# efeslab/Atom

Measured on AMD Instinct MI355X. Metric: effective TOPS, W4A4 group-128 GEMM + 128 INT8 outlier cols, fp16 out, higher is better.
Workload: dtype int4xint4 exact integer dot (BF6-coded on the f8f6f4 MFMA; INT8 MFMA for the keeper), fp32 dequant, fp16 out

## Files before the change

### atom_amd/csrc/gemm_w4a4_f6.hip

```cpp
#include <type_traits>
#include "common.h"
#include "quant_math.h"

namespace atom {

__global__ void splitk_reduce_kernel(const float *ws, half_t *D, int64_t MN, int splits);

namespace f6 {

typedef const __attribute__((address_space(1))) void *gptr_t;
typedef __attribute__((address_space(3))) void *lptr_t;
typedef int v8i __attribute__((ext_vector_type(8)));
typedef float v16f __attribute__((ext_vector_type(16)));

constexpr int TN = 2;
constexpr int PITCH = 104;
constexpr float kMagic = 12582912.0f;
constexpr int kMagicBits = 0x4B400000;

template <int BM_, int BN_, int TM_, int NS_, int OCC_ = 2, int FS_ = 0>
struct Cfg {
  static constexpr int FS = FS_;
  static constexpr int FS32 = FS_ == 1;
  static constexpr int OCC = OCC_;
// ... 221 lines not shown
      for (int q = 0; q < 4; ++q) sbp[q] = *reinterpret_cast<const v2u *>(psb + (tn * 32 + 8 * q) * 2);
#pragma unroll
      for (int r = 0; r < 16; ++r) {
        const half_t *hv = reinterpret_cast<const half_t *>(&sbp[r >> 2]);
        const float idot = __int_as_float(a[r]) - kMagic;
        c[tn][tm][r] = __builtin_fmaf(idot, (float)hv[r & 3] * sa, c[tn][tm][r]);
        asm volatile("" : "+v"(c[tn][tm][r]));
      }
    }
  }
}

template <class C, bool SK, int ABL = 0>
__global__ __launch_bounds__(C::NT, C::OCC) void gemm_w4a4_f6_kernel(GemmParams p) {
  extern __shared__ __attribute__((aligned(16))) char lds[];
  constexpr int TM = C::TM, NS = C::NS;
  const int tid = threadIdx.x;
  const int lane = tid & 63;
  const int wave = __builtin_amdgcn_readfirstlane(tid >> 6);
  __builtin_assume(wave >= 0 && wave < C::NW);
  const int wm = wave / C::WGN, wn = wave % C::WGN;

  const int nbn = (p.N + C::BN - 1) / C::BN, nbm = (p.M + C::BM - 1) / C::BM;
  const int nwg = nbm * nbn;
  int id = blockIdx.x;
  {
    const int q = nwg >> 3, r = nwg & 7, xcd = id & 7, k = id >> 3;
    id = (xcd < r ? xcd * (q + 1) : r * (q + 1) + (xcd - r) * q) + k;
  }
  constexpr int GM = 4;
  const int band = id / (GM * nbn), inband = id % (GM * nbn);
  const int rows_in_band = min(GM, nbm - band * GM);
  const int bm = band * GM + inband % rows_in_band, bn = inband / rows_in_band;
  const int m0 = bm * C::BM, n0 = bn * C::BN;

  float c[TN][TM][16];
#pragma unroll
  for (int a = 0; a < TN; ++a)
#pragma unroll
    for (int b = 0; b < TM; ++b)
#pragma unroll
      for (int r = 0; r < 16; ++r) c[a][b][r] = 0.f;

  const int csteps = p.G + 1;
  const int s_begin = SK ? (int)((int64_t)csteps * blockIdx.y / p.splits) : 0;
  const int c_end = SK ? (int)((int64_t)csteps * (blockIdx.y + 1) / p.splits) : csteps;
  const bool has_keeper = c_end == csteps;
  const int nsteps = c_end + (has_keeper ? 1 : 0);
  auto issue = [&](int step) {
    char *slot = lds + (step % NS) * C::STAGE_BYTES;
    const int s = min(step, nsteps - 1);
    if (wave >= C::NDW) return;
    if (s < p.G) issue_int4<C>(p, s, slot, wave, lane, m0, n0);
    else issue_keeper<C>(p, s - p.G, slot, wave, lane, m0, n0);
  };
#pragma unroll
  for (int s = 0; s < NS - 1; ++s) issue(s_begin + s);
  unsigned long long *tbase = nullptr;
  if constexpr ((ABL & 16) != 0)
    if (blockIdx.x == 0 && lane == 0) tbase = reinterpret_cast<unsigned long long *>(p.Dsz) + wave * 64 * 8;
#define ATOM_F6_STAMP(k) if constexpr ((ABL & 16) != 0) { if (tbase) tbase[step * 8 + k] = __builtin_amdgcn_s_memtime(); }
#define ATOM_F6_STEP(ISSUE, COMPUTE)                                                     \
  {                                                                                      \
    ATOM_F6_STAMP(0)                                                                     \
    asm volatile("s_waitcnt vmcnt(%0)" ::"n"((ABL & 1) ? 0 : C::GLDS * (NS - 2)) : "memory"); \
    ATOM_F6_STAMP(1)                                                                     \
    __builtin_amdgcn_s_barrier();                                                        \
    ATOM_F6_STAMP(2)                                                                     \
    ISSUE;                                                                               \
    __builtin_amdgcn_sched_barrier(0);                                                   \
    COMPUTE;                                                                             \
  }
  int step = s_begin;
  for (; step + NS - 1 < min(p.G, nsteps); ++step) {
    char *nslot = lds + ((step + NS - 1) % NS) * C::STAGE_BYTES;
    const int g = step + NS - 1;
    auto dma = [&](int i) { if (!(ABL & 1) && wave < C::NDW) issue_int4_piece<C>(p, g, nslot, wave, lane, m0, n0, i); };
    ATOM_F6_STEP((void)0, (compute_int4<C, ABL>(lds + (step % NS) * C::STAGE_BYTES, wm, wn, lane, c, dma, tbase ? tbase + step * 8 : nullptr, wave < C::NW / 2)))
  }
  for (; step < min(p.G, nsteps); ++step)
    ATOM_F6_STEP(if (!(ABL & 1)) issue(step + NS - 1), (compute_int4<C, ABL>(lds + (step % NS) * C::STAGE_BYTES, wm, wn, lane, c, NoDma(), nullptr, wave < C::NW / 2)))
  __builtin_amdgcn_s_setprio(0);
#undef ATOM_F6_STEP
  if (has_keeper) {
    asm volatile("s_waitcnt vmcnt(0)" ::: "memory");
    __builtin_amdgcn_s_barrier();
    if constexpr (NS == 2) {
      if (wave < C::NDW) issue_keeper<C>(p, 1, lds + ((p.G + 1) % NS) * C::STAGE_BYTES, wave, lane, m0, n0);
      asm volatile("s_waitcnt vmcnt(0)" ::: "memory");
      __builtin_amdgcn_s_barrier();
    }
    compute_keeper<C>(lds + (p.G % NS) * C::STAGE_BYTES, lds + ((p.G + 1) % NS) * C::STAGE_BYTES, wm, wn, lane, c);
    ++step;
  }
  { ATOM_F6_STAMP(0) }
  asm volatile("s_waitcnt vmcnt(0)" ::: "memory");
  __builtin_amdgcn_s_barrier();

  const int l31 = lane & 31, h = lane >> 5;
  if constexpr (SK) {
    float *wsp = p.ws + (int64_t)blockIdx.y * p.M * p.N;
#pragma unroll
    for (int tm = 0; tm < TM; ++tm) {
      const int m = m0 + wm * C::WM + tm * 32 + l31;
      if (m >= p.M) continue;
#pragma unroll
      for (int tn = 0; tn < TN; ++tn)
#pragma unroll
        for (int q = 0; q < 4; ++q) {
          const int n = n0 + wn * 64 + tn * 32 + 8 * q + 4 * h;
          if (n >= p.N) continue;
          *reinterpret_cast<v4f *>(wsp + (int64_t)m * p.N + n) =
              v4f{c[tn][tm][4 * q], c[tn][tm][4 * q + 1], c[tn][tm][4 * q + 2], c[tn][tm][4 * q + 3]};
        }
    }
    return;
  }
  constexpr int EP_STRIDE = 144;
  char *ep = lds + wave * (64 * EP_STRIDE);
#pragma unroll
  for (int half = 0; half < TM / 2; ++half) {
#pragma unroll
    for (int t2 = 0; t2 < 2; ++t2) {
      const int tm = half * 2 + t2;
#pragma unroll
      for (int tn = 0; tn < TN; ++tn)
#pragma unroll
        for (int q = 0; q < 4; ++q) {
          v2u o;
          half_t *ov = reinterpret_cast<half_t *>(&o);
#pragma unroll
          for (int k = 0; k < 4; ++k) ov[k] = f2h(c[tn][tm][4 * q + k]);
          *reinterpret_cast<v2u *>(ep + (t2 * 32 + l31) * EP_STRIDE + (tn * 32 + 8 * q + 4 * h) * 2) = o;
        }
    }
#pragma unroll
    for (int i = 0; i < 8; ++i) {
      const int rl = i * 8 + (lane >> 3);
      const int ch = lane & 7;
      const v4u v = *reinterpret_cast<const v4u *>(ep + rl * EP_STRIDE + ch * 16);
      const int m = m0 + wm * C::WM + half * 64 + rl;
      const int n = n0 + wn * 64 + ch * 8;
      if (m < p.M && n < p.N) *reinterpret_cast<v4u *>(p.D + (int64_t)m * p.N + n) = v;
    }
  }
}

typedef float v4f_t __attribute__((ext_vector_type(4)));

template <bool PAIR, bool INTER = true>
__device__ __forceinline__ void deq_pair(const v4f_t &a0, const v4f_t &a1, float sa, const float *sb, float (&c0)[4], float (&c1)[4]) {
  if constexpr (PAIR) {
    static_assert(INTER, "shared products need the interleaved rows");
    float s[4];
#pragma unroll
    for (int r = 0; r < 4; ++r) s[r] = sa * sb[r];
#pragma unroll
    for (int r = 0; r < 4; ++r) { c0[r] = __builtin_fmaf(a0[r], s[r], c0[r]); asm volatile("" : "+v"(c0[r])); }
#pragma unroll
    for (int r = 0; r < 4; ++r) { c1[r] = __builtin_fmaf(a1[r], s[r], c1[r]); asm volatile("" : "+v"(c1[r])); }
  } else if constexpr (INTER) {
    float s[8];
#pragma unroll
    for (int k = 0; k < 2; ++k)
#pragma unroll
      for (int r = 0; r < 4; ++r) s[4 * k + r] = sa * sb[2 * r + k];
#pragma unroll
    for (int r = 0; r < 4; ++r) { c0[r] = __builtin_fmaf(a0[r], s[r], c0[r]); asm volatile("" : "+v"(c0[r])); }
#pragma unroll
    for (int r = 0; r < 4; ++r) { c1[r] = __builtin_fmaf(a1[r], s[4 + r], c1[r]); asm volatile("" : "+v"(c1[r])); }
  } else {
    float s[4];
#pragma unroll
    for (int r = 0; r < 4; ++r) s[r] = sa * sb[r];
#pragma unroll
    for (int r = 0; r < 4; ++r) { c0[r] = __builtin_fmaf(a0[r], s[r], c0[r]); asm volatile("" : "+v"(c0[r])); }
#pragma unroll
    for (int r = 0; r < 4; ++r) s[r] = sa * sb[4 + r];
#pragma unroll
    for (int r = 0; r < 4; ++r) { c1[r] = __builtin_fmaf(a1[r], s[r], c1[r]); asm volatile("" : "+v"(c1[r])); }
  }
}

__device__ __forceinline__ void dequant4x(const v4f_t &acc, float sa, const v2u &sb, float (&c)[4]) {
  const half_t *hv = reinterpret_cast<const half_t *>(&sb);
  float t[4];
#pragma unroll
  for (int r = 0; r < 4; ++r) t[r] = (float)hv[r] * sa;
#pragma unroll
  for (int r = 0; r < 4; ++r) {
    c[r] = __builtin_fmaf(acc[r], t[r], c[r]);
    asm volatile("" : "+v"(c[r]));
  }
}

template <class C, class F = NoDma, bool PRIO = (C::NW >= 8), bool PH = false>
__device__ __forceinline__ void compute_int4_x16(const char *slot, int wm, int wn, int lane, float (&c)[4][C::WM / 16][4], F dma = F(),
                                                 bool older = false, unsigned *tp = nullptr) {
  const int l15 = lane & 15, kb = lane >> 4;
  const char *pw = slot + (wn * 64 + l15) * PITCH + kb * 24;
  constexpr int NTB = C::WM / 16;
  const char *pa = slot + C::A_OFF + (wm * C::WM + l15) * PITCH + kb * 24;
  const char *psa = slot + C::A_OFF + (wm * C::WM + l15) * PITCH + 96;
  const char *psb = slot + C::SB_OFF + (wn * 64 + 4 * kb) * (C::FS32 ? 4 : 2);
  v8i af[4], bf[2];
  using sa_t = typename std::conditional<C::FS != 0, float, half_t>::type;
  using sb_t = typename std::conditional<C::FS != 0, v4f_t, v2u>::type;
  constexpr int SA_AT = C::FS ? 4 : 0;
  sb_t sb[4];
  bf[0] = frag24(pa);
  af[0] = frag24(pw);
  sa_t sah = *reinterpret_cast<const sa_t *>(psa + SA_AT);
#pragma unroll
  for (int fb = 1; fb < 4; ++fb) af[fb] = frag24(pw + fb * 16 * PITCH);
#pragma unroll
  for (int fb = 0; fb < 4; ++fb) {
    if constexpr (C::FS == 2) {
      const v2u raw = *reinterpret_cast<const v2u *>(psb + fb * 32);
      const half_t *hv = reinterpret_cast<const half_t *>(&raw);
      sb[fb] = v4f_t{(float)hv[0], (float)hv[1], (float)hv[2], (float)hv[3]};
    } else {
      sb[fb] = *reinterpret_cast<const sb_t *>(psb + fb * (C::FS32 ? 64 : 32));
    }
  }
  constexpr int GS = 2, NG = 4 * NTB / GS, GPB = 4 / GS, DEPTH = 1;
  v4f_t acc[DEPTH + 1][GS];
  auto mma = [&](int g) {
    const int tb = g / GPB, f0 = (g % GPB) * GS;
#pragma unroll
    for (int k = 0; k < GS; ++k) {
      acc[g % (DEPTH + 1)][k] = v4f_t{0.f, 0.f, 0.f, 0.f};
      if constexpr (C::FS)
        acc[g % (DEPTH + 1)][k] = __builtin_amdgcn_mfma_scale_f32_16x16x128_f8f6f4(af[f0 + k], bf[tb & 1], acc[g % (DEPTH + 1)][k], 3, 3, 0, 0, 0, 0);
      else
        acc[g % (DEPTH + 1)][k] = __builtin_amdgcn_mfma_scale_f32_16x16x128_f8f6f4(af[f0 + k], bf[tb & 1], acc[g % (DEPTH + 1)][k], 3, 3, 0, 127, 0, 127);
    }
  };
  mma(0);
#ifdef ATOM_TOOLS
  if (tp) { __builtin_amdgcn_sched_barrier(0); tp[0] = (unsigned)__builtin_amdgcn_s_memtime(); }
#endif
  float sa = 0.f;
#pragma unroll
  for (int g = 0; g < NG; ++g) {
    const int tb = g / GPB, f0 = (g % GPB) * GS;
    __builtin_amdgcn_sched_barrier(0);
#ifdef ATOM_TOOLS
    if (tp && g == NG / 2) tp[1] = (unsigned)__builtin_amdgcn_s_memtime();
#endif
    if (g % GPB == 0) {
      sa = (float)sah;
      if (tb + 1 < NTB) {
        bf[(tb + 1) & 1] = frag24(pa + (tb + 1) * 16 * PITCH);
        sah = *reinterpret_cast<const sa_t *>(psa + SA_AT + (tb + 1) * 16 * PITCH);
      }
      if constexpr (PH) {
        if (tb == NTB / 2) __builtin_amdgcn_s_barrier();
      }
      if constexpr (PRIO) {
        if (tb == 0) { if (older) __builtin_amdgcn_s_setprio(0); else __builtin_amdgcn_s_setprio(2); }
        if (tb == NTB / 2) { if (older) __builtin_amdgcn_s_setprio(2); else __builtin_amdgcn_s_setprio(0); }
      }
    }
    if (g + DEPTH < NG) mma(g + DEPTH);
    if (g % GPB == GPB - 1) {
#pragma unroll
      for (int i = (tb * C::GLDS + NTB - 1) / NTB; i < ((tb + 1) * C::GLDS + NTB - 1) / NTB; ++i) dma(i);
    }
    __builtin_amdgcn_sched_barrier(0);
    {
      float w[4 * GS];
#pragma unroll
      for (int k = 0; k < GS; ++k)
#pragma unroll
        for (int r = 0; r < 4; ++r) {
          if constexpr (C::FS) w[4 * k + r] = sb[f0 + k][r];
          else w[4 * k + r] = (float)reinterpret_cast<const half_t *>(&sb[f0 + k])[r];
        }
      deq_pair<false, false>(acc[g % (DEPTH + 1)][0], acc[g % (DEPTH + 1)][1], sa, w, c[f0][tb], c[f0 + 1][tb]);
    }
  }
}

template <class C, bool PH = false>
__device__ __forceinline__ void compute_keeper_x16(const char *slot, const char *slot1, int wm, int wn, int lane, float (&c)[4][C::WM / 16][4]) {
  const int l15 = lane & 15, kb = lane >> 4;
  const int sw = (l15 >> 2) & 3;
  const int ow = (wn * 64 + l15) * 64 + ((kb ^ sw) << 4);
  constexpr int NTB = C::WM / 16;
  const int oa = (C::BN + wm * C::WM + l15) * 64 + ((kb ^ sw) << 4);
  const char *psa = slot + C::KP_SA_OFF + (wm * C::WM + l15) * 4;
  const char *psb = slot + C::SB_OFF + (wn * 64 + 4 * kb) * 2;
  v4i af[4], af1[4];
  v2u sb[4];
#pragma unroll
  for (int fb = 0; fb < 4; ++fb) {
    af[fb] = __builtin_bit_cast(v4i, *reinterpret_cast<const v4u *>(slot + ow + fb * 1024));
    af1[fb] = __builtin_bit_cast(v4i, *reinterpret_cast<const v4u *>(slot1 + ow + fb * 1024));
    sb[fb] = *reinterpret_cast<const v2u *>(psb + fb * 32);
  }
#pragma unroll
  for (int tb = 0; tb < NTB; ++tb) {
    if constexpr (PH) {
      if (tb == NTB / 2) __builtin_amdgcn_s_barrier();
    }
    const v4i b = __builtin_bit_cast(v4i, *reinterpret_cast<const v4u *>(slot + oa + tb * 1024));
    const v4i b1 = __builtin_bit_cast(v4i, *reinterpret_cast<const v4u *>(slot1 + oa + tb * 1024));
    const float sa = (float)*reinterpret_cast<const half_t *>(psa + tb * 64);
#pragma unroll
    for (int fb = 0; fb < 4; ++fb) {
      v4i a = {0, 0, 0, 0};
      a = __builtin_amdgcn_mfma_i32_16x16x64_i8(af[fb], b, a, 0, 0, 0);
      a = __builtin_amdgcn_mfma_i32_16x16x64_i8(af1[fb], b1, a, 0, 0, 0);
      const v4f_t f = {(float)a[0], (float)a[1], (float)a[2], (float)a[3]};
      dequant4x(f, sa, sb[fb], c[fb][tb]);
    }
  }
}

template <class C, int KG>
__device__ __forceinline__ void kg_exchange_store(const GemmParams &p, char *lds_all, float (&c)[4][C::WM / 16][4], int kg, int wave, int wm,
                                                  int wn, int lane, int m0, int n0) {
  constexpr int NTB = C::WM / 16, EP_STRIDE = 144;
  const int l15 = lane & 15, kb = lane >> 4;
  const int wave_all = kg * C::NW + wave;
  constexpr int HB = NTB / 2, XF = HB * 16;
  float *xw = reinterpret_cast<float *>(lds_all + C::NW * KG * (HB * 16 * EP_STRIDE)) + (kg * C::NW + wave) * XF * 64 + lane;
  const float *xr = reinterpret_cast<const float *>(lds_all + C::NW * KG * (HB * 16 * EP_STRIDE)) + ((1 - kg) * C::NW + wave) * XF * 64 + lane;
#pragma unroll
  for (int h = 0; h < 2; ++h)
    if (h != kg) {
#pragma unroll
      for (int t = 0; t < HB; ++t)
#pragma unroll
// ... 449 lines not shown
    const int q = nwg >> 3, r = nwg & 7, xcd = id & 7, k = id >> 3;
    id = (xcd < r ? xcd * (q + 1) : r * (q + 1) + (xcd - r) * q) + k;
  }
  constexpr int GM = 4;
  const int band = id / (GM * nbn), inband = id % (GM * nbn);
  const int rows_in_band = min(GM, nbm - band * GM);
  const int bm = band * GM + inband % rows_in_band, bn = inband / rows_in_band;
  const int m0 = bm * C::BM, n0 = bn * C::BN;

  float c[4][8][4];
#pragma unroll
  for (int a = 0; a < 4; ++a)
#pragma unroll
    for (int b = 0; b < 8; ++b)
#pragma unroll
      for (int r = 0; r < 4; ++r) c[a][b][r] = 0.f;

  const int G = p.G;
  auto slot_of = [&](int stage) { return lds + (stage % 3) * C::STAGE_BYTES; };
  auto issue = [&](int stage) {
    if (stage < G) issue_int4<C>(p, stage, slot_of(stage), wave, lane, m0, n0);
    else if (stage < G + 2) issue_keeper<C>(p, stage - G, slot_of(stage), wave, lane, m0, n0);
  };
  issue(0);
  issue(1);
  kstamp(1);
  asm volatile("s_waitcnt vmcnt(%0)" ::"n"(C::GLDS) : "memory");
  __builtin_amdgcn_s_barrier();
  kstamp(2);
  const int l15 = lane & 15, kb = lane >> 4;
  PRegs<C> R;
  R.lo[0] = l15 * (2 * PITCH) + kb * 24;
  R.lo[1] = R.lo[0] + 8;
  R.lo[2] = R.lo[0] + 16;
  asm volatile("" : "+v"(R.lo[1]));
  asm volatile("" : "+v"(R.lo[2]));
  {
    const char *slot = slot_of(0);
    const char *pw = slot + wn * 64 * PITCH, *pa = slot + C::A_OFF + wm * 128 * PITCH;
    const char *psa = pa + l15 * (2 * PITCH) + 96;
    R.bf[2] = frag3<C>(R, pa, p_row(0) * PITCH);
#pragma unroll
    for (int fb = 0; fb < 4; ++fb) R.af[fb] = frag3<C>(R, pw, p_row(fb) * PITCH);
    R.bf[1] = frag3<C>(R, pa, p_row(1) * PITCH);
    R.bf[0] = R.bf[1];
    R.sah[2] = *reinterpret_cast<const half_t *>(psa + p_row(0) * PITCH);
    R.sah[1] = *reinterpret_cast<const half_t *>(psa + p_row(1) * PITCH);
    R.sah[0] = (half_t)0;
    p_load_sb<C>(R, slot, wn, kb);
    p_cvt_sb<C>(R, 0);
    p_cvt_sb<C>(R, 1);
#pragma unroll
    for (int k = 0; k < 2; ++k) R.acc[1][k] = v4f_t{0.f, 0.f, 0.f, 0.f};
#pragma unroll
    for (int t = 0; t < 8; ++t) R.sa[t] = 0.f;
  }
  auto sync = [&]() {
    asm volatile("s_waitcnt vmcnt(0)" ::: "memory");
    if constexpr (!(ABL & 512)) __builtin_amdgcn_s_barrier();
  };
  {
    int s = 0;
    auto dma4 = [&](int i) { if (i < C::GLDS) issue_int4_piece<C>(p, s + 2, slot_of(s + 2), wave, lane, m0, n0, i); };
    auto dmak0 = [&](int i) { if (i == 0) issue_keeper<C>(p, 0, slot_of(G), wave, lane, m0, n0); };
    auto dmak1 = [&](int i) { if (i == 0) issue_keeper<C>(p, 1, slot_of(G + 1), wave, lane, m0, n0); };
    auto tr_sel = [&]() {
      if constexpr ((ABL & 16) != 0) {
        if (tr_on) tr_i += 6;
        tr_on = blockIdx.x == 0 && tr_i + 6 <= 78 && (s < 3 || s == G / 2 || s == G / 2 + 1 || s + 3 >= G);
      }
    };
    kstamp(3);
    if constexpr ((ABL & 1024) != 0) {
      auto dma4f = [&](int i) { if (i < C::GLDS) issue_int4_piece<C>(p, s + 2, lds + 2 * C::STAGE_BYTES, wave, lane, m0, n0, i); };
      for (; s + 2 < G; ++s) p_step<C, false, ABL>(R, lds, lds + C::STAGE_BYTES, wm, wn, lane, c, sync, dma4f, stamp);
    }
    for (; s + 2 < G; ++s) { tr_sel(); p_step<C, false, ABL>(R, slot_of(s), slot_of(s + 1), wm, wn, lane, c, sync, dma4, stamp); }
    if (G >= 2) { tr_sel(); p_step<C, false, ABL>(R, slot_of(s), slot_of(s + 1), wm, wn, lane, c, sync, dmak0, stamp); ++s; }
    tr_sel();
    p_step<C, true, ABL>(R, slot_of(s), slot_of(s + 1), wm, wn, lane, c, sync, dmak1, stamp);
  }
  kstamp(4);
  p_drain<C>(R, c);
  kstamp(5);
  asm volatile("s_waitcnt vmcnt(0)" ::: "memory");
  __builtin_amdgcn_s_barrier();
  kstamp(6);
  if constexpr (!(ABL & 128)) p_keeper<C>(slot_of(G), slot_of(G + 1), wm, wn, lane, c);
  kstamp(7);

#pragma unroll
  for (int tb = 0; tb < 8; ++tb) {
    const int m = m0 + wm * 128 + p_row(tb) + 2 * l15;
    if (m >= p.M) continue;
#pragma unroll
    for (int h = 0; h < 2; ++h) {
      const int n = n0 + wn * 64 + 32 * h + 8 * kb;
      if (n >= p.N) continue;
      v4u o;
      half_t *ov = reinterpret_cast<half_t *>(&o);
#pragma unroll
      for (int r = 0; r < 4; ++r) {
        ov[2 * r] = f2h(c[2 * h][tb][r]);
        ov[2 * r + 1] = f2h(c[2 * h + 1][tb][r]);
      }
      if constexpr ((ABL & 64) != 0) { if (o.x != 0x12345678u) continue; }
      *reinterpret_cast<v4u *>(p.D + (int64_t)m * p.N + n) = o;
    }
  }
  if constexpr ((ABL & 16) != 0) {
    kstamp(8);
    asm volatile("s_waitcnt vmcnt(0)" ::: "memory");
    kstamp(9);
    if (blockIdx.x == 0) {
      if (lane == 0) trl[79] = (unsigned)__builtin_amdgcn_s_memrealtime();
      asm volatile("s_waitcnt lgkmcnt(0)" ::: "memory");
      for (int i = lane; i < 80; i += 64) reinterpret_cast<unsigned *>(p.Dsz)[wave * 80 + i] = trl[i];
    }
  }
}

template <class C>
struct QC {
  static constexpr int SB_OFF = C::SB_OFF;
  static constexpr int STAGE = C::SB_OFF + C::BN * 4;
  static constexpr int LDS_BYTES = 3 * STAGE;
  static_assert(LDS_BYTES <= 160 * 1024 && STAGE + (32 * 3 + 1) * PITCH + 100 < 65536, "q kernel: stage layout / ds offsets");
};

typedef float v2f_t __attribute__((ext_vector_type(2)));
#ifdef ATOM_SA_B32
struct QSa {
  float v;
  __device__ __forceinline__ QSa() = default;
  __device__ __forceinline__ QSa(float f) : v(f) {}
  __device__ __forceinline__ operator float() const { return v; }
};
#else
struct QSa {
  v2f_t p;
  __device__ __forceinline__ QSa() = default;
  __device__ __forceinline__ QSa(float f) : p{0.f, f} {}
  __device__ __forceinline__ QSa(v2f_t q) : p(q) {}
  __device__ __forceinline__ operator float() const { asm volatile("" ::"v"(p)); return p.y; }
};
#endif

template <class C, bool PAIR = false, bool SA2 = false>
struct QRegs {
  v8i af[4];
  v8i bf[3];
  float sb[2][PAIR ? 4 : 8];
  QSa sa[4];
  v2f_t sa2[2];
  v4f_t acc[2][2];
  int aW[2][3], aA[2][3], aS[2], aB[2];
  int aS2[3][4];
  __device__ __forceinline__ float tscale(int tb) const {
    if constexpr (SA2) return sa2[(tb & 3) >> 1][tb & 1];
    else return sa[tb & 3];
  }
#ifdef ATOM_F6_PAIR128
  int aWp[2][3];
#endif
};

template <int SL> __device__ __forceinline__ constexpr int q_set() { return SL == 2 ? 1 : 0; }
template <class C, int SL> __device__ __forceinline__ constexpr int q_imm() { return SL == 1 ? QC<C>::STAGE : 0; }

template <class T>
__device__ __forceinline__ T q_ld0(int a, int imm) {
#if defined(__HIP_DEVICE_COMPILE__)
  typedef const __attribute__((address_space(3))) char *cp_t;
  typedef const __attribute__((address_space(3))) T *tp_t;
  return *(tp_t)((cp_t)(unsigned)a + imm);
#else
  return T{};
#endif
}
template <class C, int SL, bool Z = false>
__device__ __forceinline__ v8i q_frag(const char *lds, const int (&a)[2][3], int off, int ro) {
  const char *b = lds + (SL < 0 ? ro : q_imm<C, SL>()) + off;
  v2u x, y, z;
  if constexpr (Z) {
    const int imm = (SL < 0 ? 0 : q_imm<C, SL>()) + off, r = SL < 0 ? ro : 0;
    x = q_ld0<v2u>(a[q_set<SL>()][0] + r, imm);
    y = q_ld0<v2u>(a[q_set<SL>()][1] + r, imm);
    z = q_ld0<v2u>(a[q_set<SL>()][2] + r, imm);
  } else {
    x = *reinterpret_cast<const v2u *>(b + a[q_set<SL>()][0]);
    y = *reinterpret_cast<const v2u *>(b + a[q_set<SL>()][1]);
    z = *reinterpret_cast<const v2u *>(b + a[q_set<SL>()][2]);
  }
  asm volatile("" ::: "memory");
  return v8i{(int)x.x, (int)x.y, (int)y.x, (int)y.y, (int)z.x, (int)z.y, 0, 0};
}
#ifdef ATOM_F6_PAIR128
template <class C, int SL>
__device__ __forceinline__ void q_frag_pair(const char *lds, const int (&a)[2][3], int off, int ro, v8i &f0, v8i &f1) {
  const char *b = lds + (SL < 0 ? ro : q_imm<C, SL>()) + off;
  const v4u x = *reinterpret_cast<const v4u *>(b + a[q_set<SL>()][0]);
  const v4u y = *reinterpret_cast<const v4u *>(b + a[q_set<SL>()][1]);
  const v4u z = *reinterpret_cast<const v4u *>(b + a[q_set<SL>()][2]);
  asm volatile("" ::: "memory");
  f0 = v8i{(int)x.x, (int)x.y, (int)y.x, (int)y.y, (int)z.x, (int)z.y, 0, 0};
  f1 = v8i{(int)x.z, (int)x.w, (int)y.z, (int)y.w, (int)z.z, (int)z.w, 0, 0};
}
#endif
template <class C, int SL, class RG>
__device__ __forceinline__ QSa q_scale(const char *lds, const RG &R, int off, int ro) {
#ifdef ATOM_SA_B32
  return *reinterpret_cast<const float *>(lds + (SL < 0 ? ro : q_imm<C, SL>()) + off + R.aS[q_set<SL>()] + 4);
#else
  return QSa(*reinterpret_cast<const v2f_t *>(lds + (SL < 0 ? ro : q_imm<C, SL>()) + off + R.aS[q_set<SL>()]));
#endif
}
template <class C, int SL, class RG>
__device__ __forceinline__ v2f_t q_scale2(const char *lds, const RG &R, int j, int ro) {
  const int a = R.aS2[SL < 0 ? 0 : SL][j] + (SL < 0 ? ro : 0);
  return v2f_t{q_ld0<float>(a, 100), q_ld0<float>(a, PITCH + 100)};
}
template <class C, int SL, class RG>
__device__ __forceinline__ void q_load_sb(const char *lds, RG &R, int h, int ro) {
  const char *b = lds + (SL < 0 ? ro : q_imm<C, SL>()) + QC<C>::SB_OFF + 128 * h + R.aB[q_set<SL>()];
  if constexpr (sizeof(R.sb[0]) == 4 * sizeof(float)) {
    const float *f = reinterpret_cast<const float *>(b);
#pragma unroll
    for (int k = 0; k < 4; ++k) R.sb[h][k] = f[2 * k];
  } else {
    const v4f_t lo = *reinterpret_cast<const v4f_t *>(b), hi = *reinterpret_cast<const v4f_t *>(b + 16);
#pragma unroll
    for (int k = 0; k < 4; ++k) { R.sb[h][k] = lo[k]; R.sb[h][4 + k] = hi[k]; }
  }
}

__device__ __forceinline__ void q_dma16x3(unsigned m0v, unsigned voff, const void *sbase) {
  asm volatile("s_mov_b32 m0, %0\n\ts_nop 0\n\tglobal_load_lds_dwordx4 %1, %2\n\tglobal_load_lds_dwordx4 %1, %2 offset:1024\n\t"
               "global_load_lds_dwordx4 %1, %2 offset:2048" ::"s"(m0v), "v"(voff), "s"(sbase) : "memory");
}
__device__ __forceinline__ void q_dma16(unsigned m0v, unsigned voff, const void *sbase) {
  asm volatile("s_mov_b32 m0, %0\n\ts_nop 0\n\tglobal_load_lds_dwordx4 %1, %2" ::"s"(m0v), "v"(voff), "s"(sbase) : "memory");
}
struct QDma {
  unsigned voffW, voffA, voffX;
  int m0W, m0A, m0X;
  int xkind;
};
template <class C, int DS>
__device__ __forceinline__ void q_piece(const QDma &d, const uint8_t *wsrc, const uint8_t *asrc, const float *sbsrc, int i) {
  constexpr int base = DS * QC<C>::STAGE;
  if (i == 0) q_dma16x3(base + d.m0W, d.voffW, wsrc);
  else if (i == 3) q_dma16x3(base + d.m0A, d.voffA, asrc);
  else if (i == 6) {
    const void *xb = d.xkind == 1 ? (const void *)wsrc : (d.xkind == 2 ? (const void *)asrc : (const void *)sbsrc);
    q_dma16(base + d.m0X, d.voffX, xb);
  }
}

struct QNoEarly { __device__ __forceinline__ void operator()(int) const {} };
template <class C, int SL, bool PAIR, bool SA2, class FS, class FD, class FE = QNoEarly>
__device__ __forceinline__ void q_step(QRegs<C, PAIR, SA2> &R, const char *lds, float (&c)[4][8][4], FS sync, FD mid, int ro = 0, int rn = 0,
                                       bool LAST = false, FE early = FE(), unsigned *tp = nullptr) {
  constexpr int NX = SL < 0 ? -1 : (SL + 1) % 3;
  auto stamp = [&](int k) {
    if (tp) { __builtin_amdgcn_sched_barrier(0); const unsigned t_ = (unsigned)__builtin_amdgcn_s_memtime(); if ((threadIdx.x & 63) == 0) tp[k] = t_; __builtin_amdgcn_sched_barrier(0); }
  };
#pragma unroll
  for (int i = 0; i < 16; ++i) {
    const int tb = p_tb(i), h = p_h(i);
    __builtin_amdgcn_sched_barrier(0);
    stamp(i);
    if (i == 8) { stamp(16); sync(); stamp(17); }
    __builtin_amdgcn_sched_barrier(0);
#pragma unroll
    for (int k = 0; k < 2; ++k)
      R.acc[i & 1][k] = __builtin_amdgcn_mfma_scale_f32_16x16x128_f8f6f4(R.af[2 * h + k], R.bf[p_buf(tb)], v4f_t{0.f, 0.f, 0.f, 0.f}, 3, 3, 0, 0, 0, 0);
    __builtin_amdgcn_sched_barrier(0);
    stamp(32 + 2 * i);
    if (h == 1 && i < 12 && tb + 2 < 8) {
      R.bf[p_buf(tb + 2)] = q_frag<C, SL, SA2>(lds, R.aA, p_row(tb + 2) * PITCH, ro);
      if constexpr (SA2) {
        if ((tb & 1) == 0) R.sa2[((tb + 2) & 3) >> 1] = q_scale2<C, SL>(lds, R, (tb + 2) >> 1, ro);
      } else R.sa[(tb + 2) & 3] = q_scale<C, SL>(lds, R, p_row(tb + 2) * PITCH, ro);
    }
    if (!LAST) {
      if (i == 12) {
        R.bf[2] = q_frag<C, NX, SA2>(lds, R.aA, p_row(0) * PITCH, rn);
        if constexpr (!SA2) R.sa[0] = q_scale<C, NX>(lds, R, p_row(0) * PITCH, rn);
      }
      if (i == 13) {
#ifdef ATOM_F6_PAIR128
        q_frag_pair<C, NX>(lds, R.aWp, p_row(0) * PITCH, rn, R.af[0], R.af[1]);
#else
        R.af[0] = q_frag<C, NX, SA2>(lds, R.aW, p_row(0) * PITCH, rn);
        R.af[1] = q_frag<C, NX, SA2>(lds, R.aW, p_row(1) * PITCH, rn);
#endif
      }
      if (i == 15) {
#ifdef ATOM_F6_PAIR128
        q_frag_pair<C, NX>(lds, R.aWp, p_row(2) * PITCH, rn, R.af[2], R.af[3]);
#else
        R.af[2] = q_frag<C, NX, SA2>(lds, R.aW, p_row(2) * PITCH, rn);
        R.af[3] = q_frag<C, NX, SA2>(lds, R.aW, p_row(3) * PITCH, rn);
#endif
        R.bf[1] = q_frag<C, NX, SA2>(lds, R.aA, p_row(1) * PITCH, rn);
        if constexpr (!SA2) R.sa[1] = q_scale<C, NX>(lds, R, p_row(1) * PITCH, rn);
      }
      if constexpr (SA2) { if (i == 14) R.sa2[0] = q_scale2<C, NX>(lds, R, 0, rn); }
    }
    if (i >= 8) mid(i - 8);
    else early(i);
    if (tp) asm volatile("s_waitcnt lgkmcnt(0)" ::: "memory");
    stamp(33 + 2 * i);
    __builtin_amdgcn_sched_barrier(0);
    {
      const int j = (i + 15) & 15, dtb = p_tb(j), dh = p_h(j);
      deq_pair<PAIR>(R.acc[j & 1][0], R.acc[j & 1][1], R.tscale(dtb), R.sb[dh], c[2 * dh][dtb], c[2 * dh + 1][dtb]);
    }
    __builtin_amdgcn_sched_barrier(0);
    if (!LAST && i == 14) q_load_sb<C, NX>(lds, R, 0, rn);
    if (i == 0) q_load_sb<C, SL>(lds, R, 1, ro);
  }
  stamp(18);
}

template <class C, bool STORE, int NTB, bool WHOLE = false>
__device__ __forceinline__ void q_keeper(const GemmParams &p, const char *slot, const char *slot1, int wm, int wn, int lane, float (&c)[4][NTB][4],
                                         int m0, int n0) {
  constexpr bool MERGED = true;
  const int l15 = lane & 15, kb = lane >> 4;
  const int sw = (l15 >> 1) & 3;
  const char *pw = slot + (wn * 64 + 2 * l15) * 64 + ((kb ^ sw) << 4);
  const char *pa = slot + (C::BN + wm * (16 * NTB) + 2 * l15) * 64 + ((kb ^ sw) << 4);
  const char *psa = slot + C::KP_SA_OFF + (wm * (16 * NTB) + 2 * l15) * 4;
  const char *psb = slot + C::SB_OFF + (wn * 64 + 8 * kb) * 2;
  v4i af[4], bf[2];
  v4i af1[4], bf1[2];
  const long d1 = slot1 - slot;
  float sb[2][8], sa[2];
  v4i acc[2][2];
  const v4i magic = {kMagicBits, kMagicBits, kMagicBits, kMagicBits};
#pragma unroll
  for (int fb = 0; fb < 4; ++fb) af[fb] = __builtin_bit_cast(v4i, *reinterpret_cast<const v4u *>(pw + p_row(fb) * 64));
  bf[0] = __builtin_bit_cast(v4i, *reinterpret_cast<const v4u *>(pa + p_row(0) * 64));
  bf[1] = __builtin_bit_cast(v4i, *reinterpret_cast<const v4u *>(pa + p_row(1) * 64));
  if constexpr (MERGED) {
#pragma unroll
    for (int fb = 0; fb < 4; ++fb) af1[fb] = __builtin_bit_cast(v4i, *reinterpret_cast<const v4u *>(pw + d1 + p_row(fb) * 64));
    bf1[0] = __builtin_bit_cast(v4i, *reinterpret_cast<const v4u *>(pa + d1 + p_row(0) * 64));
    bf1[1] = __builtin_bit_cast(v4i, *reinterpret_cast<const v4u *>(pa + d1 + p_row(1) * 64));
  }
  half_t sah[2];
  sah[0] = *reinterpret_cast<const half_t *>(psa + p_row(0) * 4);
  sah[1] = *reinterpret_cast<const half_t *>(psa + p_row(1) * 4);
#pragma unroll
  for (int h = 0; h < 2; ++h) {
    const v4u w = *reinterpret_cast<const v4u *>(psb + 64 * h);
    const half_t *hv = reinterpret_cast<const half_t *>(&w);
#pragma unroll
    for (int j = 0; j < 8; ++j) { sb[h][j] = (float)hv[j]; asm volatile("" : "+v"(sb[h][j])); }
  }
  unsigned dvoff = 0;
  if constexpr (STORE && WHOLE) {
    dvoff = (unsigned)(((wm * (16 * NTB) + 2 * l15) * p.N + wn * 64 + 8 * kb) * 2);
    asm volatile("" : "+v"(dvoff));
  }
  auto store_block = [&](int tb) {
    const int m = m0 + wm * (16 * NTB) + p_row(tb) + 2 * l15;
    if constexpr (!WHOLE) { if (m >= p.M) return; }
#pragma unroll
    for (int h = 0; h < 2; ++h) {
      const int n = n0 + wn * 64 + 32 * h + 8 * kb;
      if constexpr (!WHOLE) { if (n >= p.N) continue; }
      v4u o;
      half_t *ov = reinterpret_cast<half_t *>(&o);
#pragma unroll
      for (int r = 0; r < 4; ++r) {
        ov[2 * r] = f2h(c[2 * h][tb][r]);
        ov[2 * r + 1] = f2h(c[2 * h + 1][tb][r]);
      }
      if constexpr (WHOLE) {
        char *dtb = reinterpret_cast<char *>(p.D + ((int64_t)(m0 + p_row(tb)) * p.N + n0));
        *reinterpret_cast<v4u *>(dtb + dvoff + 64 * h) = o;
      } else {
        *reinterpret_cast<v4u *>(p.D + (int64_t)m * p.N + n) = o;
      }
    }
  };
  auto dequant = [&](int j) {
    const int tb = j >> 1, h = j & 1;
    v4f_t f[2];
#pragma unroll
    for (int k = 0; k < 2; ++k)
#pragma unroll
      for (int r = 0; r < 4; ++r) f[k][r] = __int_as_float(acc[j & 1][k][r]) - kMagic;
    deq_pair<false>(f[0], f[1], sa[tb & 1], sb[h], c[2 * h][tb], c[2 * h + 1][tb]);
  };
#pragma unroll
  for (int i = 0; i < 2 * NTB; ++i) {
    const int tb = i >> 1, h = i & 1;
    __builtin_amdgcn_sched_barrier(0);
    if (h == 0) sa[tb & 1] = (float)sah[tb & 1];
#pragma unroll
    for (int k = 0; k < 2; ++k) acc[i & 1][k] = __builtin_amdgcn_mfma_i32_16x16x64_i8(af[2 * h + k], bf[tb & 1], magic, 0, 0, 0);
    if constexpr (MERGED) {
#pragma unroll
      for (int k = 0; k < 2; ++k) acc[i & 1][k] = __builtin_amdgcn_mfma_i32_16x16x64_i8(af1[2 * h + k], bf1[tb & 1], acc[i & 1][k], 0, 0, 0);
    }
    __builtin_amdgcn_sched_barrier(0);
    if (h == 1 && tb + 2 < NTB) {
      bf[tb & 1] = __builtin_bit_cast(v4i, *reinterpret_cast<const v4u *>(pa + p_row(tb + 2) * 64));
      if constexpr (MERGED) bf1[tb & 1] = __builtin_bit_cast(v4i, *reinterpret_cast<const v4u *>(pa + d1 + p_row(tb + 2) * 64));
      sah[tb & 1] = *reinterpret_cast<const half_t *>(psa + p_row(tb + 2) * 4);
    }
    if constexpr (STORE) { if (h == 1 && tb >= 1) store_block(tb - 1); }
    __builtin_amdgcn_sched_barrier(0);
    if (i > 0) dequant(i - 1);
  }
  __builtin_amdgcn_sched_barrier(0);
  dequant(2 * NTB - 1);
  if constexpr (STORE) store_block(NTB - 1);
}

template <class C, int GU = 0, bool TR = false, bool PAIR = false>
__global__ __launch_bounds__(C::NT, C::OCC) void gemm_w4a4_f6q_kernel(GemmParams p) {
  extern __shared__ __attribute__((aligned(16))) char lds[];
  static_assert(C::BM == 256 && C::BN == 256 && C::WM == 128 && C::NS == 3 && C::NW == 8, "q kernel: 256x256, 8 waves of 64 x 128");
  using Q = QC<C>;
  unsigned *trb = nullptr;
  auto kstamp = [&](int k) {
    if constexpr (TR) {
      if (trb) { const unsigned t = (unsigned)__builtin_amdgcn_s_memtime(); if ((threadIdx.x & 63) == 0) trb[k] = t; }
    }
  };
  if constexpr (TR) {
    if (blockIdx.x == 0 || blockIdx.x == gridDim.x - 1) {
      trb = reinterpret_cast<unsigned *>(p.Dsz) + ((blockIdx.x ? 8 : 0) + (threadIdx.x >> 6)) * 128;
      if ((threadIdx.x & 63) == 0) trb[62] = (unsigned)__builtin_amdgcn_s_memrealtime();
    }
    kstamp(0);
  }
  const int tid = threadIdx.x;
  const int lane = tid & 63;
  const int wave = __builtin_amdgcn_readfirstlane(tid >> 6);
  __builtin_assume(wave >= 0 && wave < C::NW);
  const int wm = wave / C::WGN, wn = wave % C::WGN;
  const int nbn = (p.N + C::BN - 1) / C::BN, nbm = (p.M + C::BM - 1) / C::BM;
  const int nwg = nbm * nbn;
  int id = blockIdx.x;
  {
    const int q = nwg >> 3, r = nwg & 7, xcd = id & 7, k = id >> 3;
    id = (xcd < r ? xcd * (q + 1) : r * (q + 1) + (xcd - r) * q) + k;
  }
  constexpr int GM = 4;
  const int band = id / (GM * nbn), inband = id % (GM * nbn);
  const int rows_in_band = min(GM, nbm - band * GM);
  const int bm = band * GM + inband % rows_in_band, bn = inband / rows_in_band;
  const int m0 = bm * C::BM, n0 = bn * C::BN;

  float c[4][8][4];
#pragma unroll
  for (int a = 0; a < 4; ++a)
#pragma unroll
    for (int b = 0; b < 8; ++b)
#pragma unroll
      for (int r = 0; r < 4; ++r) c[a][b][r] = 0.f;

  const int G = p.G;
  QDma d;
  d.voffW = d.voffA = (unsigned)(wave * 3072 + lane * 16);
  d.m0W = wave * 3072;
  d.m0A = C::A_OFF + wave * 3072;
  d.xkind = wave < 2 ? 1 : (wave < 4 ? 2 : 3);
  d.voffX = (unsigned)((wave < 4 ? (24 + (wave & 1)) * 1024 : 0) + lane * 16);
  d.m0X = wave < 2 ? (24 + wave) * 1024 : (wave < 4 ? C::A_OFF + (24 + (wave & 1)) * 1024 : Q::SB_OFF);
  const int64_t wstep = p.f6_rows_b * PITCH, astep = p.f6_rows_a * PITCH;
  const uint8_t *wsrc0 = p.B4 + (int64_t)n0 * PITCH, *asrc0 = p.A4 + (int64_t)m0 * PITCH;
  const float *sbsrc0 = p.sB32 + n0;
  auto slot_of = [&](int stage) { return lds + (stage % 3) * Q::STAGE; };
  auto issue_all = [&](auto ds, int g) {
    constexpr int DS = decltype(ds)::value;
#pragma unroll
    for (int i = 0; i < 7; ++i) q_piece<C, DS>(d, wsrc0 + g * wstep, asrc0 + g * astep, sbsrc0 + (int64_t)g * p.f6_rows_b, i);
  };
  const bool early1 = G >= 6;
  issue_all(std::integral_constant<int, 0>(), 0);
  if (!early1) {
    if (G >= 2) issue_all(std::integral_constant<int, 1>(), 1);
    else issue_keeper<C>(p, 0, slot_of(1), wave, lane, m0, n0);
  }
  kstamp(1);
  asm volatile("s_waitcnt vmcnt(0)" ::: "memory");
  __builtin_amdgcn_s_barrier();
  kstamp(2);

  const int l15 = lane & 15, kb = lane >> 4;
#ifdef ATOM_Q_NO_SA2
  constexpr bool SA2 = false;
#else
  constexpr bool SA2 = PAIR && GU == 0;
#endif
  QRegs<C, PAIR, SA2> R;
  {
    const int lw = wn * 64 * PITCH + l15 * (2 * PITCH) + kb * 24;
    const int la = C::A_OFF + wm * 128 * PITCH + l15 * (2 * PITCH);
#pragma unroll
    for (int st = 0; st < 2; ++st) {
#pragma unroll
      for (int k = 0; k < 3; ++k) {
        R.aW[st][k] = lw + 8 * k + st * 2 * Q::STAGE;
        R.aA[st][k] = la + kb * 24 + 8 * k + st * 2 * Q::STAGE;
        asm volatile("" : "+v"(R.aW[st][k]), "+v"(R.aA[st][k]));
#ifdef ATOM_F6_PAIR128
        R.aWp[st][k] = ((wn * 64 * PITCH + l15 * (2 * PITCH) + kb * 48 + 16 * k + st * 2 * Q::STAGE) & ~15);
        asm volatile("" : "+v"(R.aWp[st][k]));
#endif
      }
      R.aS[st] = la + 96 + st * 2 * Q::STAGE;
      R.aB[st] = (wn * 64 + 8 * kb) * 4 + st * 2 * Q::STAGE;
      if constexpr (!SA2) asm volatile("" : "+v"(R.aS[st]));
      asm volatile("" : "+v"(R.aB[st]));
    }
    if constexpr (SA2) {
#pragma unroll
      for (int sl = 0; sl < 3; ++sl)
#pragma unroll
        for (int j = 0; j < 4; ++j) {
          R.aS2[sl][j] = la + sl * Q::STAGE + p_row(2 * j) * PITCH;
          asm volatile("" : "+v"(R.aS2[sl][j]));
        }
    }
    R.bf[2] = q_frag<C, 0, SA2>(lds, R.aA, p_row(0) * PITCH, 0);
#pragma unroll
    for (int fb = 0; fb < 4; ++fb) R.af[fb] = q_frag<C, 0, SA2>(lds, R.aW, p_row(fb) * PITCH, 0);
    R.bf[1] = q_frag<C, 0, SA2>(lds, R.aA, p_row(1) * PITCH, 0);
    R.bf[0] = R.bf[1];
    if constexpr (SA2) {
      R.sa2[0] = q_scale2<C, 0>(lds, R, 0, 0);
      R.sa2[1] = v2f_t{0.f, 0.f};
    } else {
      R.sa[0] = q_scale<C, 0>(lds, R, p_row(0) * PITCH, 0);
      R.sa[1] = q_scale<C, 0>(lds, R, p_row(1) * PITCH, 0);
      R.sa[2] = 0.f;
      R.sa[3] = 0.f;
    }
    q_load_sb<C, 0>(lds, R, 0, 0);
    q_load_sb<C, 0>(lds, R, 1, 0);
#pragma unroll
    for (int k = 0; k < 2; ++k) R.acc[1][k] = v4f_t{0.f, 0.f, 0.f, 0.f};
  }
  if constexpr (TR) { asm volatile("s_waitcnt lgkmcnt(0)" ::: "memory"); kstamp(3); }
  auto sync = [&]() {
    asm volatile("s_waitcnt vmcnt(0)" ::: "memory");
    __builtin_amdgcn_s_barrier();
  };
  auto reg = [&](auto sl, int s) {
    constexpr int SL = decltype(sl)::value;
#ifndef ATOM_TR_LOOP_ONLY
    if constexpr (TR) { if (s < 44) kstamp(16 + s); }
#endif
    const int g = s + 2;
    const uint8_t *wsrc = wsrc0 + g * wstep, *asrc = asrc0 + g * astep;
    const float *sbsrc = sbsrc0 + (int64_t)g * p.f6_rows_b;
    unsigned *tp = nullptr;
#ifndef ATOM_TR_LOOP_ONLY
    if constexpr (TR) { if (trb && s == 9) tp = trb + 64; }
#endif
    q_step<C, SL, PAIR>(R, lds, c, sync, [&](int i) { q_piece<C, (SL + 2) % 3>(d, wsrc, asrc, sbsrc, i); }, 0, 0, false, QNoEarly(), tp);
  };
  using S0 = std::integral_constant<int, 0>;
  using S1 = std::integral_constant<int, 1>;
  using S2 = std::integral_constant<int, 2>;
  int s = 0;
  if (early1) {
    if constexpr (TR) kstamp(16);
    const uint8_t *wsrc = wsrc0 + 2 * wstep, *asrc = asrc0 + 2 * astep;
    const float *sbsrc = sbsrc0 + (int64_t)2 * p.f6_rows_b;
    q_step<C, 0, PAIR>(R, lds, c, sync, [&](int i) { q_piece<C, 2>(d, wsrc, asrc, sbsrc, i); }, 0, 0, false,
                 [&](int i) { q_piece<C, 1>(d, wsrc0 + wstep, asrc0 + astep, sbsrc0 + p.f6_rows_b, i); });
    reg(S1(), 1);
    reg(S2(), 2);
    s = 3;
  }
  for (; s + 4 < G; s += 3) { reg(S0(), s); reg(S1(), s + 1); reg(S2(), s + 2); }
  if (s + 2 < G) { reg(S0(), s); ++s; }
  if (s + 2 < G) { reg(S1(), s); ++s; }
  for (; s < G; ++s) {
#ifndef ATOM_TR_LOOP_ONLY
    if constexpr (TR) { if (s < 44) kstamp(16 + s); }
#endif
    const int g = s + 2;
    const int dsl = g % 3;
    const uint8_t *wsrc = wsrc0 + g * wstep, *asrc = asrc0 + g * astep;
    const float *sbsrc = sbsrc0 + (int64_t)g * p.f6_rows_b;
    q_step<C, -1, PAIR>(R, lds, c, sync,
                  [&](int i) {
                    if (g < G) {
                      if (dsl == 0) q_piece<C, 0>(d, wsrc, asrc, sbsrc, i);
                      else if (dsl == 1) q_piece<C, 1>(d, wsrc, asrc, sbsrc, i);
                      else q_piece<C, 2>(d, wsrc, asrc, sbsrc, i);
                    } else if (i == 0) issue_keeper<C>(p, g - G, slot_of(g), wave, lane, m0, n0);
                  },
                  (s % 3) * Q::STAGE, ((s + 1) % 3) * Q::STAGE, s + 1 == G);
  }
  deq_pair<PAIR>(R.acc[1][0], R.acc[1][1], R.tscale(7), R.sb[1], c[2][7], c[3][7]);
  kstamp(4);
  asm volatile("s_waitcnt vmcnt(0)" ::: "memory");
  __builtin_amdgcn_s_barrier();
  kstamp(5); kstamp(6);
  if constexpr (GU == 0) {
#ifdef ATOM_Q_NO_WHOLE
    const bool whole = false;
#else
    const bool whole = m0 + C::BM <= p.M && n0 + C::BN <= p.N && p.N <= (1 << 21);
#endif
    if (whole) q_keeper<C, true, 8, true>(p, slot_of(G), slot_of(G + 1), wm, wn, lane, c, m0, n0);
    else q_keeper<C, true, 8, false>(p, slot_of(G), slot_of(G + 1), wm, wn, lane, c, m0, n0);
  } else {
    q_keeper<C, false>(p, slot_of(G), slot_of(G + 1), wm, wn, lane, c, m0, n0);
  }
  if constexpr (TR) {
    kstamp(7);
    asm volatile("s_waitcnt vmcnt(0)" ::: "memory");
    kstamp(8);
    if (trb && (threadIdx.x & 63) == 0) trb[63] = (unsigned)__builtin_amdgcn_s_memrealtime();
  }
  if constexpr (GU == 0) return;

  if constexpr (GU != 0) {
    constexpr bool SIM = GU == 1;
    float *am = reinterpret_cast<float *>(lds + ((G + 2) % 3) * Q::STAGE);
#pragma unroll
    for (int tb = 0; tb < 8; ++tb) {
      float mx = 0.f;
#pragma unroll
      for (int k = 0; k < 2; ++k)
#pragma unroll
        for (int r = 0; r < 4; ++r) {
          const float h = silu_mul<SIM>((float)f2h(c[k][tb][r]), (float)f2h(c[2 + k][tb][r]));
          c[k][tb][r] = h;
          mx = fmaxf(mx, fabsf(h));
        }
      mx = fmaxf(mx, __shfl_xor(mx, 16));
      mx = fmaxf(mx, __shfl_xor(mx, 32));
      if (kb == 0) am[wave * 128 + p_row(tb) + 2 * l15] = mx;
    }
    __syncthreads();
    const bool keeper_blk = bn == nbn - 1;
    const GateUpOut &o = p.gu;
    const int N_inter = p.N >> 1;
#pragma unroll
    for (int tb = 0; tb < 8; ++tb) {
      const int t = p_row(tb) + 2 * l15;
      const float *ap = am + wm * 4 * 128 + t;
      const float amax = fmaxf(fmaxf(ap[0], ap[128]), fmaxf(ap[256], ap[384]));
      const GroupScale gs = group_scale<SIM>(amax, keeper_blk, o.clip);
      float tr[8];
#pragma unroll
      for (int k = 0; k < 2; ++k)
#pragma unroll
        for (int r = 0; r < 4; ++r) tr[2 * r + k] = group_code<SIM>(c[k][tb][r], gs);
      const int64_t m = m0 + wm * 128 + t;
      if (m >= p.M) continue;
      const half_t sh = f2h(gs.s_store);
      if (keeper_blk) {
        *reinterpret_cast<v2u *>(o.o8 + m * kKeeper + wn * 32 + kb * 8) = pack_codes8(tr, true);
      } else {
        const v6u_t f = bf6_fields(tr);
        uint8_t *dst = o.o6 + ((int64_t)bn * o.o6_rows + m) * PITCH;
        uint8_t *d6 = dst + wn * 24 + kb * 6;
        if ((kb & 1) == 0) {
          *reinterpret_cast<unsigned *>(d6) = f[0];
          *reinterpret_cast<unsigned short *>(d6 + 4) = (unsigned short)f[1];
        } else {
          *reinterpret_cast<unsigned short *>(d6) = (unsigned short)f[0];
          *reinterpret_cast<unsigned *>(d6 + 2) = (f[0] >> 16) | (f[1] << 16);
        }
        if (wn == 0 && kb == 0) *reinterpret_cast<v2u *>(dst + 96) = f6_scale_words(__builtin_bit_cast(unsigned short, sh));
      }
      if (wn == 0 && kb == 0) store_token_scale(keeper_blk ? o.s8 : (o.s4 + (int64_t)bn * o.ld4), m, sh, o.ref_layout);
      if (o.xq) {
        v4u q;
        half_t *qv = reinterpret_cast<half_t *>(&q);
#pragma unroll
        for (int j = 0; j < 8; ++j) qv[j] = dequant_half(tr[j], gs);
        *reinterpret_cast<v4u *>(o.xq + m * N_inter + bn * 128 + wn * 32 + kb * 8) = q;
      }
    }
    return;
  }
}

template <class C, int GU = 0, bool TR = false, bool PAIR = false>
static int launch_q(const GemmParams &p, hipStream_t s) {
  static std::atomic<uint64_t> attr_done{0};
  if (ensure_max_lds(reinterpret_cast<const void *>(&gemm_w4a4_f6q_kernel<C, GU, TR, PAIR>), QC<C>::LDS_BYTES, attr_done) != ATOM_OK) return ATOM_ERR_LAUNCH;
  const int nbm = (p.M + C::BM - 1) / C::BM, nbn = (p.N + C::BN - 1) / C::BN;
  hipLaunchKernelGGL((gemm_w4a4_f6q_kernel<C, GU, TR, PAIR>), dim3((unsigned)(nbm * nbn)), dim3(C::NT), QC<C>::LDS_BYTES, s, p);
  return check_launch();
}

struct QkDma {
  unsigned voff, voffX;
  int m0W, m0A, m0X;
  int xkind;
};
__device__ __forceinline__ void q_dma4(unsigned m0v, unsigned voff, const void *sbase) {
  asm volatile("s_mov_b32 m0, %0\n\ts_nop 0\n\tglobal_load_lds_dword %1, %2" ::"s"(m0v), "v"(voff), "s"(sbase) : "memory");
}
template <class C>
__device__ __forceinline__ void qk_piece(const QkDma &d, const uint8_t *wsrc, const uint8_t *asrc, const float *sbsrc, int so, int i) {
  if (i == 0) q_dma16x3(so + d.m0W, d.voff, wsrc);
  else if (i == 1) q_dma16x3(so + d.m0A, d.voff, asrc);
  else if (i == 2) {
    if (d.xkind == 3) q_dma4(so + d.m0X, d.voffX, sbsrc);
    else q_dma16(so + d.m0X, d.voffX, d.xkind == 1 ? (const void *)wsrc : (const void *)asrc);
  }
}

template <class C>
struct QkRegs {
  v8i af[4], bf[4];
  float sb[2][8];
  QSa sa[4];
  v4f_t acc[2][2];
  int aW[2][3], aA[2][3], aS[2], aB[2];
};
template <class C, int SL, int ABL = 0, class FS, class FD, class FE = QNoEarly>
__device__ __forceinline__ void qk_step(QkRegs<C> &R, const char *lds, float (&c)[4][4][4], FS sync, FD mid, int ro = 0, int rn = 0, bool LAST = false,
                                        FE early = FE()) {
  constexpr int NX = SL < 0 ? -1 : (SL + 1) % 3;
#pragma unroll
  for (int i = 0; i < 8; ++i) {
    const int tb = i & 3, h = i >> 2;
    __builtin_amdgcn_sched_barrier(0);
    if (i == 4) sync();
    __builtin_amdgcn_sched_barrier(0);
    if constexpr (!(ABL & 4)) {
#pragma unroll
      for (int k = 0; k < 2; ++k)
        R.acc[i & 1][k] = __builtin_amdgcn_mfma_scale_f32_16x16x128_f8f6f4(R.af[2 * h + k], R.bf[tb], v4f_t{0.f, 0.f, 0.f, 0.f}, 3, 3, 0, 0, 0, 0);
    }
    __builtin_amdgcn_sched_barrier(0);
    if constexpr (!(ABL & 8)) {
      if (i == 0) {
        R.af[2] = q_frag<C, SL>(lds, R.aW, p_row(2) * PITCH, ro);
        R.af[3] = q_frag<C, SL>(lds, R.aW, p_row(3) * PITCH, ro);
      }
      if (!LAST && i >= 4) {
        if (i == 4) {
          R.af[0] = q_frag<C, NX>(lds, R.aW, p_row(0) * PITCH, rn);
          R.af[1] = q_frag<C, NX>(lds, R.aW, p_row(1) * PITCH, rn);
        }
        R.bf[tb] = q_frag<C, NX>(lds, R.aA, p_row(tb) * PITCH, rn);
      }
    }
    if (i >= 4) mid(i - 4);
    else early(i);
// ... 547 lines not shown
```

Baseline: 2763.

## Compute dequant scale outer products with a 16x16x1 f32 MFMA in SA2 path

In the SA2 dequant path, the per-lane products of activation and weight group scales are now formed by one 16x16x1 f32 MFMA outer product every four sub-steps, replacing scalar multiplies. Each lane loads a single sa and sb value instead of vectors of scales, which cuts LDS scale reads and VALU multiplies. The cost is an extra MFMA issue, 16 more accumulator registers held live, and a reworked scale addressing and load schedule. It only takes effect when the SA2 configuration is chosen.

```diff
diff --git a/atom_amd/csrc/gemm_w4a4_f6.hip b/atom_amd/csrc/gemm_w4a4_f6.hip
--- a/atom_amd/csrc/gemm_w4a4_f6.hip
+++ b/atom_amd/csrc/gemm_w4a4_f6.hip
@@ -397,9 +397,13 @@
 __device__ __forceinline__ void deq_pair(const v4f_t &a0, const v4f_t &a1, float sa, const float *sb, float (&c0)[4], float (&c1)[4]) {
   if constexpr (PAIR) {
     static_assert(INTER, "shared products need the interleaved rows");
+#ifdef ATOM_F6_SCALE4X4
+    const v4f_t s = __builtin_amdgcn_mfma_f32_4x4x1f32(sb[0], sa, v4f_t{0.f, 0.f, 0.f, 0.f}, 0, 0, 0);
+#else
     float s[4];
 #pragma unroll
     for (int r = 0; r < 4; ++r) s[r] = sa * sb[r];
+#endif
 #pragma unroll
     for (int r = 0; r < 4; ++r) { c0[r] = __builtin_fmaf(a0[r], s[r], c0[r]); asm volatile("" : "+v"(c0[r])); }
 #pragma unroll
@@ -425,6 +429,17 @@
 #pragma unroll
     for (int r = 0; r < 4; ++r) { c1[r] = __builtin_fmaf(a1[r], s[r], c1[r]); asm volatile("" : "+v"(c1[r])); }
   }
+}
+
+typedef float v16f_t __attribute__((ext_vector_type(16)));
+__device__ __forceinline__ v16f_t scale_tile4(float sb_lane, float sa_lane) {
+  return __builtin_amdgcn_mfma_f32_16x16x1f32(sb_lane, sa_lane, v16f_t{0.f, 0.f, 0.f, 0.f, 0.f, 0.f, 0.f, 0.f, 0.f, 0.f, 0.f, 0.f, 0.f, 0.f, 0.f, 0.f}, 0, 0, 0);
+}
+__device__ __forceinline__ void deq_pair_t(const v4f_t &a0, const v4f_t &a1, const v16f_t &t, int b, float (&c0)[4], float (&c1)[4]) {
+#pragma unroll
+  for (int r = 0; r < 4; ++r) { c0[r] = __builtin_fmaf(a0[r], t[4 * b + r], c0[r]); asm volatile("" : "+v"(c0[r])); }
+#pragma unroll
+  for (int r = 0; r < 4; ++r) { c1[r] = __builtin_fmaf(a1[r], t[4 * b + r], c1[r]); asm volatile("" : "+v"(c1[r])); }
 }
 
 __device__ __forceinline__ void dequant4x(const v4f_t &acc, float sa, const v2u &sb, float (&c)[4]) {
@@ -1180,14 +1195,13 @@
   v8i bf[3];
   float sb[2][PAIR ? 4 : 8];
   QSa sa[4];
-  v2f_t sa2[2];
+  float sbq[2];
+  float saq;
+  v16f_t st;
   v4f_t acc[2][2];
   int aW[2][3], aA[2][3], aS[2], aB[2];
-  int aS2[3][4];
-  __device__ __forceinline__ float tscale(int tb) const {
-    if constexpr (SA2) return sa2[(tb & 3) >> 1][tb & 1];
-    else return sa[tb & 3];
-  }
+  int aSq[2][2], aBq[2][2];
+  __device__ __forceinline__ float tscale(int tb) const { return sa[tb & 3]; }
 #ifdef ATOM_F6_PAIR128
   int aWp[2][3];
 #endif
@@ -1244,9 +1258,12 @@
 #endif
 }
 template <class C, int SL, class RG>
-__device__ __forceinline__ v2f_t q_scale2(const char *lds, const RG &R, int j, int ro) {
-  const int a = R.aS2[SL < 0 ? 0 : SL][j] + (SL < 0 ? ro : 0);
-  return v2f_t{q_ld0<float>(a, 100), q_ld0<float>(a, PITCH + 100)};
+__device__ __forceinline__ float q_scale_q(const RG &R, int q, int ro) {
+  return q_ld0<float>(R.aSq[q_set<SL>()][q == 3] + (SL < 0 ? ro : 0), (SL < 0 ? 0 : q_imm<C, SL>()) + (q == 3 ? 96 : 32 * q) * PITCH + 100);
+}
+template <class C, int SL, class RG>
+__device__ __forceinline__ float q_load_sbq(const RG &R, int k, int ro) {
+  return q_ld0<float>(R.aBq[q_set<SL>()][k] + (SL < 0 ? ro : 0), SL < 0 ? 0 : q_imm<C, SL>());
 }
 template <class C, int SL, class RG>
 __device__ __forceinline__ void q_load_sb(const char *lds, RG &R, int h, int ro) {
@@ -1307,10 +1324,9 @@
     stamp(32 + 2 * i);
     if (h == 1 && i < 12 && tb + 2 < 8) {
       R.bf[p_buf(tb + 2)] = q_frag<C, SL, SA2>(lds, R.aA, p_row(tb + 2) * PITCH, ro);
-      if constexpr (SA2) {
-        if ((tb & 1) == 0) R.sa2[((tb + 2) & 3) >> 1] = q_scale2<C, SL>(lds, R, (tb + 2) >> 1, ro);
-      } else R.sa[(tb + 2) & 3] = q_scale<C, SL>(lds, R, p_row(tb + 2) * PITCH, ro);
-    }
+      if constexpr (!SA2) R.sa[(tb + 2) & 3] = q_scale<C, SL>(lds, R, p_row(tb + 2) * PITCH, ro);
+    }
+    if constexpr (SA2) { if ((i & 3) == 2 && i < 14) R.saq = q_scale_q<C, SL>(R, (i + 2) >> 2, ro); }
     if (!LAST) {
       if (i == 12) {
         R.bf[2] = q_frag<C, NX, SA2>(lds, R.aA, p_row(0) * PITCH, rn);
@@ -1334,7 +1350,11 @@
         R.bf[1] = q_frag<C, NX, SA2>(lds, R.aA, p_row(1) * PITCH, rn);
         if constexpr (!SA2) R.sa[1] = q_scale<C, NX>(lds, R, p_row(1) * PITCH, rn);
       }
-      if constexpr (SA2) { if (i == 14) R.sa2[0] = q_scale2<C, NX>(lds, R, 0, rn); }
+      if constexpr (SA2) {
+        if (i == 14) R.saq = q_scale_q<C, NX>(R, 0, rn);
+        if (i == 10) R.sbq[0] = q_load_sbq<C, NX>(R, 0, rn);
+        if (i == 13) R.sbq[1] = q_load_sbq<C, NX>(R, 1, rn);
+      }
     }
     if (i >= 8) mid(i - 8);
     else early(i);
@@ -1343,11 +1363,16 @@
     __builtin_amdgcn_sched_barrier(0);
     {
       const int j = (i + 15) & 15, dtb = p_tb(j), dh = p_h(j);
-      deq_pair<PAIR>(R.acc[j & 1][0], R.acc[j & 1][1], R.tscale(dtb), R.sb[dh], c[2 * dh][dtb], c[2 * dh + 1][dtb]);
+      if constexpr (SA2) deq_pair_t(R.acc[j & 1][0], R.acc[j & 1][1], R.st, j & 3, c[2 * dh][dtb], c[2 * dh + 1][dtb]);
+      else deq_pair<PAIR>(R.acc[j & 1][0], R.acc[j & 1][1], R.tscale(dtb), R.sb[dh], c[2 * dh][dtb], c[2 * dh + 1][dtb]);
     }
     __builtin_amdgcn_sched_barrier(0);
-    if (!LAST && i == 14) q_load_sb<C, NX>(lds, R, 0, rn);
-    if (i == 0) q_load_sb<C, SL>(lds, R, 1, ro);
+    if constexpr (SA2) {
+      if ((i & 3) == 0) { R.st = scale_tile4(R.sbq[i == 12], R.saq); __builtin_amdgcn_sched_barrier(0); }
+    } else {
+      if (!LAST && i == 14) q_load_sb<C, NX>(lds, R, 0, rn);
+      if (i == 0) q_load_sb<C, SL>(lds, R, 1, ro);
+    }
   }
   stamp(18);
 }
@@ -1551,11 +1576,12 @@
     }
     if constexpr (SA2) {
 #pragma unroll
-      for (int sl = 0; sl < 3; ++sl)
-#pragma unroll
-        for (int j = 0; j < 4; ++j) {
-          R.aS2[sl][j] = la + sl * Q::STAGE + p_row(2 * j) * PITCH;
-          asm volatile("" : "+v"(R.aS2[sl][j]));
+      for (int st = 0; st < 2; ++st)
+#pragma unroll
+        for (int k = 0; k < 2; ++k) {
+          R.aSq[st][k] = la + (k ? (kb & 1) : (kb >> 1)) * PITCH + st * 2 * Q::STAGE;
+          R.aBq[st][k] = Q::SB_OFF + (wn * 64 + 32 * (k ? (kb >> 1) : (kb & 1)) + 2 * l15) * 4 + st * 2 * Q::STAGE;
+          asm volatile("" : "+v"(R.aSq[st][k]), "+v"(R.aBq[st][k]));
         }
     }
     R.bf[2] = q_frag<C, 0, SA2>(lds, R.aA, p_row(0) * PITCH, 0);
@@ -1564,16 +1590,20 @@
     R.bf[1] = q_frag<C, 0, SA2>(lds, R.aA, p_row(1) * PITCH, 0);
     R.bf[0] = R.bf[1];
     if constexpr (SA2) {
-      R.sa2[0] = q_scale2<C, 0>(lds, R, 0, 0);
-      R.sa2[1] = v2f_t{0.f, 0.f};
+      R.saq = q_scale_q<C, 0>(R, 0, 0);
+      R.sbq[0] = q_load_sbq<C, 0>(R, 0, 0);
+      R.sbq[1] = q_load_sbq<C, 0>(R, 1, 0);
+      R.st = scale_tile4(R.sbq[1], 0.f);
     } else {
       R.sa[0] = q_scale<C, 0>(lds, R, p_row(0) * PITCH, 0);
       R.sa[1] = q_scale<C, 0>(lds, R, p_row(1) * PITCH, 0);
       R.sa[2] = 0.f;
       R.sa[3] = 0.f;
     }
-    q_load_sb<C, 0>(lds, R, 0, 0);
-    q_load_sb<C, 0>(lds, R, 1, 0);
+    if constexpr (!SA2) {
+      q_load_sb<C, 0>(lds, R, 0, 0);
+      q_load_sb<C, 0>(lds, R, 1, 0);
+    }
 #pragma unroll
     for (int k = 0; k < 2; ++k) R.acc[1][k] = v4f_t{0.f, 0.f, 0.f, 0.f};
   }
@@ -1631,7 +1661,8 @@
                   },
                   (s % 3) * Q::STAGE, ((s + 1) % 3) * Q::STAGE, s + 1 == G);
   }
-  deq_pair<PAIR>(R.acc[1][0], R.acc[1][1], R.tscale(7), R.sb[1], c[2][7], c[3][7]);
+  if constexpr (SA2) deq_pair_t(R.acc[1][0], R.acc[1][1], R.st, 3, c[2][7], c[3][7]);
+  else deq_pair<PAIR>(R.acc[1][0], R.acc[1][1], R.tscale(7), R.sb[1], c[2][7], c[3][7]);
   kstamp(4);
   asm volatile("s_waitcnt vmcnt(0)" ::: "memory");
   __builtin_amdgcn_s_barrier();
```

Result: faster. 2802, median of 6 (+1.4%).
